# mzhaoshuai/CenterCLIP

Hardware: AMD Instinct MI355X
Metric: clips/sec (ViT-B/32, 12f) (higher is better)
Workload: dtype fp16 (MFMA operands; fp32 accumulate, residual stream, LN, softmax; cluster + similarity fp32); 1 GPU; cfg2 MSR-VTT-shaped: ViT-B/32 224^2, 12 frames -> 3 segments @block 7, K=49, batch 16, 32 words; global_batch=16, parallelism=single GPU

## Files before the change

### centerclip_amd/_lib_clip.py

```python
import ctypes as c

CC_MAX_LAYERS = 32
EPI = {"f16": 0, "f16_gelu": 1, "f32_resid": 2, "f32": 4}


class BlockWeights(c.Structure):
    _fields_ = [(n, c.c_void_p) for n in (
        "ln_1_weight", "ln_1_bias", "in_proj_weight_f16", "in_proj_bias", "out_proj_weight_f16", "out_proj_bias",
        "ln_2_weight", "ln_2_bias", "c_fc_weight_f16", "c_fc_bias", "c_proj_weight_f16", "c_proj_bias",
        "in_proj_ln_weight_f16", "in_proj_ln_c1", "in_proj_ln_c2", "c_fc_ln_weight_f16", "c_fc_ln_c1", "c_fc_ln_c2")]


class VitModel(c.Structure):
    _fields_ = [("layers", c.c_int32), ("width", c.c_int32), ("heads", c.c_int32), ("patch", c.c_int32),
                ("resolution", c.c_int32), ("embed_dim", c.c_int32),
                ("conv1_weight_f16", c.c_void_p), ("class_embedding", c.c_void_p),
                ("positional_embedding", c.c_void_p), ("ln_pre_weight", c.c_void_p), ("ln_pre_bias", c.c_void_p),
                ("ln_post_weight", c.c_void_p), ("ln_post_bias", c.c_void_p), ("proj", c.c_void_p),
                ("blocks", c.POINTER(BlockWeights)),
                ("cluster_frames", c.c_int32 * CC_MAX_LAYERS), ("cluster_tokens", c.c_int32 * CC_MAX_LAYERS),
                ("cluster_metric", c.c_int32), ("cluster_norm_p", c.c_float), ("cluster_threshold", c.c_float),
                ("cluster_iter_limit", c.c_int32), ("cluster_split_size", c.c_int32), ("cluster_pre_norm", c.c_int32),
                ("cluster_variants", c.c_void_p), ("row_policy", c.c_int32), ("conv2_weight_f16", c.c_void_p)]


class Frames(c.Structure):
    _fields_ = [("data", c.c_void_p), ("format", c.c_int32), ("mean", c.c_float * 3), ("std", c.c_float * 3)]


class TextModel(c.Structure):
    _fields_ = [("layers", c.c_int32), ("width", c.c_int32), ("heads", c.c_int32), ("context_length", c.c_int32),
                ("vocab_size", c.c_int32), ("embed_dim", c.c_int32),
                ("token_embedding", c.c_void_p), ("positional_embedding", c.c_void_p),
                ("ln_final_weight", c.c_void_p), ("ln_final_bias", c.c_void_p), ("text_projection", c.c_void_p),
                ("blocks", c.POINTER(BlockWeights)), ("row_policy", c.c_int32)]


ROWS_ALL_TEXT, ROWS_ALL_LAST_BLOCK = 1, 2


def declare(lib):
    vp, i32, i64, f32, sz = c.c_void_p, c.c_int32, c.c_int64, c.c_float, c.c_size_t
    lib.cc_linear_f16.argtypes = [vp, vp, vp, vp, i32, i32, i32, i32, i32, i32, vp]
    lib.cc_layernorm_f32.argtypes = [vp, i64, vp, vp, vp, i64, i32, i32, f32, i32, vp]
    lib.cc_attention_f16.argtypes = [vp, vp, i32, i32, i32, i32, i32, vp]
    lib.cc_fold_layernorm_linear_f32.argtypes = [vp, vp, vp, vp, i32, i32, vp, vp, vp, vp]
    lib.cc_fold_layernorm_linear_f32.restype = c.c_int
    lib.cc_row_stats_f16.argtypes = [vp, vp, vp, vp, i32, i32, vp]
    lib.cc_linear_ln_f16.argtypes = [vp, vp, vp, vp, vp, i32, f32, vp, i32, i32, i32, i32, i32, vp]
    lib.cc_linear_resid_stats_f16.argtypes = [vp, vp, vp, vp, vp, vp, c.POINTER(i32), vp, vp, i32, vp, i32, i32, i32, i32, vp]
    lib.cc_inproj_attention_f16.argtypes = [vp, vp, vp, vp, vp, i32, f32, vp, i32, i32, i32, i32, vp, vp, vp, vp]
    lib.cc_inproj_attention_f16.restype = c.c_int
    lib.cc_linear_tile_for.argtypes = [i32, i32, i32, i32]
    lib.cc_linear_tile_for.restype = c.c_int
    lib.cc_linear_resid_stats_slots.argtypes = [i32, i32, i32, i32]
    lib.cc_linear_resid_stats_slots.restype = c.c_int
    lib.cc_attention_strided_f16.argtypes = [vp, vp, i32, i32, i32, i32, i32, i64, i64, vp]
    lib.cc_attention_strided_f16.restype = c.c_int
    lib.cc_text_encode_hidden.argtypes = [c.POINTER(TextModel), vp, i32, i32, vp, vp, vp, sz, vp]
    lib.cc_text_encode_hidden.restype = c.c_int
    lib.cc_head_project_f32.argtypes = [vp, i32, vp, vp, vp, vp, vp, i32, i32, i32, vp]
    lib.cc_head_project_f32.restype = c.c_int
    lib.cc_contrastive_loss_f32.argtypes = [vp, i32, i64, i64, vp, vp, sz, vp]
    lib.cc_contrastive_loss_f32.restype = c.c_int
    lib.cc_contrastive_grad_workspace_bytes.argtypes = [i32, i32, i32]
    lib.cc_contrastive_grad_workspace_bytes.restype = sz
    lib.cc_contrastive_loss_grad_f32.argtypes = [vp, vp, vp, i64, i64, i32, i32, i32, f32, f32, vp, vp, vp, vp, vp, sz, vp]
    lib.cc_contrastive_loss_grad_f32.restype = c.c_int
    lib.cc_contrastive_loss_grad_dev_f32.argtypes = [vp, vp, vp, i64, i64, i32, i32, i32, f32, vp, f32, vp, vp, vp, vp, vp, sz, vp]
    lib.cc_contrastive_loss_grad_dev_f32.restype = c.c_int
    lib.cc_normalize_rows_f32.argtypes = [vp, vp, i32, i32, vp]
    lib.cc_normalize_rows_f32.restype = c.c_int
    lib.cc_loose_similarity_grouped_f32.argtypes = [vp, vp, vp, i32, i64, i64, i64, i64, i32, i32, i32, i32, f32, vp, i32,
                                                    vp, vp, sz, vp]
    lib.cc_loose_similarity_grouped_f32.restype = c.c_int
    for name in ("cc_row_stats_f16", "cc_linear_ln_f16", "cc_linear_resid_stats_f16"):
        getattr(lib, name).restype = c.c_int
    lib.cc_rank_counts_f32.argtypes = [vp, i32, i32, i64, i64, i32, vp, vp]
    lib.cc_rank_counts_f32.restype = c.c_int
    lib.cc_rank_counts_cols_f32.argtypes = [vp, i32, i32, i64, i64, vp, vp, vp]
    lib.cc_rank_counts_cols_f32.restype = c.c_int
# ... 118 lines not shown
```

### centerclip_amd/clip.py

```python
import contextlib
import ctypes
import torch
from torch import nn

import os

from . import _lib as L
from . import ops
from . import torch_ops as T
from ._lib_clip import BlockWeights, TextModel, VitModel, CC_MAX_LAYERS, ROWS_ALL_TEXT, ROWS_ALL_LAST_BLOCK
from .cluster import get_cluster_inter


PIXEL_MEAN = (0.48145466, 0.4578275, 0.40821073)
PIXEL_STD = (0.26862954, 0.26130258, 0.27577711)


def frames_descriptor(x, mean=PIXEL_MEAN, std=PIXEL_STD):
    from ._lib_clip import Frames
    fr = Frames()
    if x.dtype == torch.uint8:
        if x.ndim != 4 or (x.shape[1] != 3 and x.shape[-1] != 3):
            raise ValueError("uint8 frames must be [N,3,H,W] or [N,H,W,3], got %s" % (tuple(x.shape),))
        x = x.contiguous()
# ... 104 lines not shown
        out = self.resblocks((x, video_frame, cluster_loss))
        return out if visual else out[0]


class _Pack:

    def __init__(self):
        self.key = None
        self.keep = []
        self.struct = None
        self.handle = None

    @staticmethod
    def signature(module):
        return tuple((p.data_ptr(), p._version, str(p.device), p.dtype) for p in module.parameters())

    def f32(self, t):
        t = t.detach().float().contiguous()
        self.keep.append(t)
        return t.data_ptr()

    def f16(self, t):
        t = t.detach().to(torch.float16).contiguous()
        self.keep.append(t)
        return t.data_ptr()

    def fold(self, linear_w, linear_b, ln):
        w = linear_w.detach().float().contiguous()
        b = linear_b.detach().float().contiguous()
        gamma, beta = ln.weight.detach().float().contiguous(), ln.bias.detach().float().contiguous()
        N, K = w.shape
        wf = torch.empty(N, K, device=w.device, dtype=torch.float16)
        c1 = torch.empty(N, device=w.device, dtype=torch.float32)
        c2 = torch.empty(N, device=w.device, dtype=torch.float32)
        L.check(L.lib().cc_fold_layernorm_linear_f32(L.ptr(w), L.ptr(b), L.ptr(gamma), L.ptr(beta), N, K, L.ptr(wf),
                                                     L.ptr(c1), L.ptr(c2), L.stream_ptr(w.device)),
                "cc_fold_layernorm_linear_f32")
        self.keep += [wf, c1, c2]
        return wf.data_ptr(), c1.data_ptr(), c2.data_ptr()

    def blocks(self, transformer, count=None):
        arr = (BlockWeights * len(transformer.resblocks))()
        for i, blk in enumerate(transformer.resblocks):
            if count is not None and i >= count:
                break
            b = arr[i]
# ... 53 lines not shown
            (("prefix", int(n_blocks)),)
        if getattr(self, "_prefix_pack", None) is None:
            self._prefix_pack = _Pack()
        return self._build(self._prefix_pack, sig, int(n_blocks))

    def _build(self, pk, sig, n_blocks):
        if pk.key == sig:
            return pk.handle
        if pk.handle is not None:
            T.release_model(pk.handle)
        pk.keep, pk.key = [], sig
        m = VitModel()
        m.row_policy = ROWS_ALL_LAST_BLOCK if self.all_last_block_rows else 0
        m.layers, m.width, m.heads = self.transformer.layers, self.width, self.heads
        m.patch, m.resolution, m.embed_dim = self.patch_size, self.input_resolution, self.output_dim
        m.conv1_weight_f16 = pk.f16(self.conv1.weight.reshape(self.width, -1))
        if self.linear_patch == '3d':
            m.conv2_weight_f16 = pk.f16(self.conv2.weight.reshape(self.width, -1))
        m.class_embedding, m.positional_embedding = pk.f32(self.class_embedding), pk.f32(self.positional_embedding)
        m.ln_pre_weight, m.ln_pre_bias = pk.f32(self.ln_pre.weight), pk.f32(self.ln_pre.bias)
        if n_blocks is None:
            m.ln_post_weight, m.ln_post_bias = pk.f32(self.ln_post.weight), pk.f32(self.ln_post.bias)
            m.proj = pk.f32(self.proj)
        m.blocks = ctypes.cast(pk.blocks(self.transformer, n_blocks), ctypes.POINTER(BlockWeights))
        first = None
        tokens = (self.input_resolution // self.patch_size) ** 2
        variants = (L.ClusterVariant * CC_MAX_LAYERS)()
        any_variant = False
        dev = self.proj.device
        for i, blk in enumerate(self.transformer.resblocks):
            tc = blk.tokencluster_inter
            if tc is not None and tc.is_shift:
                m.cluster_frames[i], m.cluster_tokens[i] = tc.original_frame, tokens
                variants[i], keep = tc.variant(tokens, dev)
                pk.keep.extend(keep)
                any_variant = True
            elif tc is not None:
                m.cluster_frames[i], m.cluster_tokens[i] = tc.after_block_frames, tc.cluster_num
                if tc.algorithm == 'pooling' and tc.cluster_num != tokens:
                    raise ValueError("'pooling' keeps the token count: cluster_num_blocks[%d] must be %d" % (i, tokens))
                if getattr(tc, "mean_residual", False) and tc.cluster_num != tokens:
                    raise ValueError("mean_residual keeps the token count (cluster.py:229): cluster_num_blocks[%d] must be %d"
                                     % (i, tokens))
                variants[i], keep = tc.variant(tc.frame_duration * tokens, dev)
                pk.keep.extend(keep)
                any_variant = any_variant or not tc.is_default_variant
# ... 178 lines not shown
            hidden = hidden.view(h.shape[0], h.shape[1], -1)
            return hidden[:, 0, :], hidden
        feats, _ = self.visual.encode(image, video_frame)
        return feats, zero_scalar(image.device)

    def _text_model(self):
        tower = nn.ModuleList([self.transformer, self.token_embedding, self.ln_final])
        sig = _Pack.signature(tower) + ((self.positional_embedding._version, self.text_projection._version,
                                         self.positional_embedding.data_ptr(), self.text_projection.data_ptr(),
                                         bool(self.all_text_rows), bool(self.all_last_block_rows)),)
        pk = self._text_pack
        if pk.key == sig:
            return pk.handle
        if pk.handle is not None:
            T.release_model(pk.handle)
        pk.keep, pk.key = [], sig
        m = TextModel()
        m.row_policy = (ROWS_ALL_TEXT if self.all_text_rows else 0) | (ROWS_ALL_LAST_BLOCK if self.all_last_block_rows else 0)
        m.layers, m.width, m.heads = self.transformer.layers, self.transformer.width, self.transformer.heads
        m.context_length, m.vocab_size, m.embed_dim = self.context_length, self.vocab_size, self.embed_dim
        m.token_embedding, m.positional_embedding = pk.f32(self.token_embedding.weight), pk.f32(self.positional_embedding)
        m.ln_final_weight, m.ln_final_bias = pk.f32(self.ln_final.weight), pk.f32(self.ln_final.bias)
        m.text_projection = pk.f32(self.text_projection)
        m.blocks = ctypes.cast(pk.blocks(self.transformer), ctypes.POINTER(BlockWeights))
        pk.struct = m
        pk.handle = T.register_model(m, dict(embed_dim=self.embed_dim, width=self.transformer.width), pk)
        return pk.handle

    def text_prefix_parameters(self, n_blocks):
        ps = [self.token_embedding.weight, self.positional_embedding]
        for blk in list(self.transformer.resblocks)[:n_blocks]:
            ps += list(blk.parameters())
        return ps

    def _text_prefix_model(self, n_blocks):
        sig = tuple((p.data_ptr(), p._version, str(p.device), p.dtype) for p in self.text_prefix_parameters(n_blocks)) + \
            (("prefix", int(n_blocks)),)
        if getattr(self, "_text_prefix_pack", None) is None:
            self._text_prefix_pack = _Pack()
        pk = self._text_prefix_pack
        if pk.key == sig:
            return pk.handle
        if pk.handle is not None:
            T.release_model(pk.handle)
        pk.keep, pk.key = [], sig
        m = TextModel()
# ... 99 lines not shown
```

### centerclip_amd/csrc/cc_kernels.h

```cpp
#pragma once
#include "cc_common.h"

enum { EPI_F16 = 0, EPI_F16_GELU = 1, EPI_F32_RESID = 2, EPI_F32_PATCH = 3, EPI_F32 = 4,
       EPI_F16_LN = 5, EPI_F16_GELU_LN = 6, EPI_F32_RESID_STATS = 7,
       EPI_ATTN_LN = 8 };
#define CC_LN_MAX_SLOTS 32

struct GemmArgs {
    const _Float16* A;
    const _Float16* W;
    const float* bias;
    void* C;
    const float* R;
    const float* pos;
    int M, N, K, ldc;
    int lda, ldw;
    int patch_n;
    int tiles_m, tiles_n;
    const float* ln_stats;
    const float* ln_c1;
    int ln_slots;
    float ln_eps;
    float* stats_out;
    _Float16* c16;
    const float* shift_in;
    const float* shift_stats;
    int shift_slots;
    float* shift_out;
    const int* m_dev;
    int row_step;
    const int* row_map;
    float out_scale;
    int n_valid;
    const float* out_unscale_dev;
    int att_L, att_nseq, att_spt, att_causal;
    const int* att_seq_off;
    const int* att_seq_len;
};

struct GemmPair {
    GemmArgs p[2];
    int tiles0;
    int rider_prio;
};

int cc_gemm_dispatch(GemmArgs g, int epi, int tile, hipStream_t st);
int cc_gemm_dispatch2(GemmArgs g0, const GemmArgs* g1, int epi, int tile, hipStream_t st, int* slots_out = nullptr);
bool cc_gemm_timing_claim(const int rec12[12], hipEvent_t* start, hipEvent_t* stop);
bool cc_gemm_rows_ok(int N, int K, int epi);
int cc_gemm_rows_dispatch2(GemmArgs g0, const GemmArgs* g1, int epi, hipStream_t st, int* slots_out = nullptr);

struct LnArgs {
    const float* in; int64_t in_stride; const float* gamma; const float* beta; void* out; int64_t out_stride;
    int rows, W;
    _Float16* out16;
    float* stats;
    float* shift;
    const float* cls;
    const float* pos0;
    int cls_period;
};
struct TextEmbedArgs {
    const long long* ids; const float* tok_emb; const float* pos; float* h; int* eot; int Bt, Lt, W;
    _Float16* h16;
    float* stats;
    float* shift;
    int* seq_off;
    int* seq_len;
    int* m_total;
    int vocab;
};
int cc_launch_row_stats(const float* h, _Float16* h16, float* stats, float* shift, int rows, int W, hipStream_t st);
int cc_launch_layernorm2(const LnArgs& a0, const LnArgs* a1, float eps, int out_f16, hipStream_t st);
// ... 44 lines not shown
```

### centerclip_amd/csrc/clip_forward.hip

```cpp
#include "cc_kernels.h"
#include <cstdlib>
#include <cstdint>

namespace {

bool is_shift(const cc_cluster_variant* var) {
    return var && (var->algorithm == CC_CLUSTER_TEMPORAL_SHIFT || var->algorithm == CC_CLUSTER_TOKEN_SHIFT);
}

struct Carver {
    char* base;
    size_t off = 0;
    explicit Carver(void* b) : base(static_cast<char*>(b)) {}
    template <typename T>
    T* take(size_t count) {
        T* ptr = base ? reinterpret_cast<T*>(base + off) : nullptr;
        off += cc_align_up(count * sizeof(T), 256);
        return ptr;
    }
};

struct VitWs {
    _Float16* im2col;
    float* h;
// ... 46 lines not shown
    v.cluster = c.take<char>(cb);
    v.total = c.off;
    return v;
}

struct BlockCtx {
    float* h;
    _Float16* h16;
    float* st0;
    float* st1;
    float* sh0;
    float* sh1;
    _Float16* qkv;
    _Float16* att;
    _Float16* u;
    int nseq, L, W, heads, causal;
    int slots0, slots1;
    const int* m_dev;
    const int* seq_off;
    const int* seq_len;
    int sel_rows, sel_step;
    const int* sel_map;
    int mid_shift, mid_seg, mid_div;
};

int run_block_pair(const cc_block_weights* w0, BlockCtx* c0, const cc_block_weights* w1, BlockCtx* c1,
                   hipStream_t st) {
    if (!w0) { w0 = w1; c0 = c1; w1 = nullptr; c1 = nullptr; }
    const int M0 = c0->nseq * c0->L, M1 = c1 ? c1->nseq * c1->L : 0;
    const int Wa = c0->W, Wb = c1 ? c1->W : 0;
    int rc;
    int slots[2];
#ifdef CC_DEV_KNOBS
    static const int unpair_mask = [] { const char* e = getenv("CC_UNPAIR"); return e ? atoi(e) : 0; }();
#else
    constexpr int unpair_mask = 0;
#endif
    const int unpair = (c1 && M0 < 5000) ? unpair_mask : 0;
    auto dispatch = [&](GemmArgs& g0, GemmArgs& g1, int epi, int bit, int* sl) {
        if (!(unpair & bit)) return cc_gemm_dispatch2(g0, c1 ? &g1 : nullptr, epi, 0, st, sl);
        int s0[2] = {0, 0}, s1[2] = {0, 0};
        int r = cc_gemm_dispatch2(g0, nullptr, epi, 0, st, sl ? s0 : nullptr);
        if (r) return r;
        r = cc_gemm_dispatch2(g1, nullptr, epi, 0, st, sl ? s1 : nullptr);
        if (sl) { sl[0] = s0[0]; sl[1] = s1[0]; }
        return r;
    };
    auto base = [&](const BlockCtx* c, int M, const _Float16* A, const void* Wt, const float* bias, void* C, int N, int K) {
        GemmArgs g{};
        g.A = A; g.W = static_cast<const _Float16*>(Wt); g.bias = bias; g.C = C;
        g.M = M; g.N = N; g.K = K; g.ldc = N;
        g.ln_eps = 1e-5f;
        g.m_dev = c->m_dev;
        return g;
    };
    auto tail = [&](const BlockCtx* c, int M, const _Float16* A, const void* Wt, const float* bias, void* C, int N, int K) {
        GemmArgs g = base(c, M, A, Wt, bias, C, N, K);
        if (c->sel_rows > 0) { g.M = c->sel_rows; g.m_dev = nullptr; g.row_step = c->sel_step; g.row_map = c->sel_map; }
        return g;
    };
    auto tail_dispatch = [&](GemmArgs& g0, GemmArgs& g1, int epi, int bit, int* sl) {
        const bool s0 = c0->sel_rows > 0, s1 = c1 && c1->sel_rows > 0;
        if (!s0 && !s1) return dispatch(g0, g1, epi, bit, sl);
        if (s0 && (s1 || !c1)) return cc_gemm_rows_dispatch2(g0, c1 ? &g1 : nullptr, epi, st, sl);
        int a[2] = {0, 0}, b[2] = {0, 0};
        int* pa = sl ? a : nullptr;
        int* pb = sl ? b : nullptr;
        int r = s0 ? cc_gemm_rows_dispatch2(g0, nullptr, epi, st, pa) : cc_gemm_dispatch2(g0, nullptr, epi, 0, st, pa);
        if (r) return r;
        r = s1 ? cc_gemm_rows_dispatch2(g1, nullptr, epi, st, pb) : cc_gemm_dispatch2(g1, nullptr, epi, 0, st, pb);
        if (sl) { sl[0] = a[0]; sl[1] = b[0]; }
        return r;
    };
    {
        GemmArgs g0 = base(c0, M0, c0->h16, w0->in_proj_ln_weight_f16, w0->in_proj_ln_c2, c0->qkv, 3 * Wa, Wa);
        g0.ln_stats = c0->st0; g0.ln_slots = c0->slots0; g0.ln_c1 = w0->in_proj_ln_c1;
        GemmArgs g1{};
        if (c1) {
            g1 = base(c1, M1, c1->h16, w1->in_proj_ln_weight_f16, w1->in_proj_ln_c2, c1->qkv, 3 * Wb, Wb);
            g1.ln_stats = c1->st0; g1.ln_slots = c1->slots0; g1.ln_c1 = w1->in_proj_ln_c1;
        }
// ... 113 lines not shown
bool text_ok(const cc_text_model* m, int Lt) {
    return m->layers > 0 && m->layers <= CC_MAX_LAYERS && m->width == m->heads * 64 && Lt <= m->context_length;
}

int encode_towers(const cc_vit_model* vm, const cc_frames* video, int B, int T, float* vfeat, float* hidden_out,
                  int64_t* medoids_out, const int64_t* forced_medoids, const cc_text_model* tm, const int64_t* ids,
                  int Bt, int Lt, float* tfeat, float* text_hidden_out, void* ws, size_t ws_bytes, hipStream_t st,
                  int vstop = -1, int tstop = -1) {
    VitWs v{};
    TextWs t{};
    size_t off = 0;
    if (vm) { v = carve_vit(vm, B, T, ws); off = v.total; }
    if (tm) { t = carve_text(tm, Bt, Lt, static_cast<char*>(ws) + off); off += t.total; }
    if (!ws || ws_bytes < off) return CC_ERR_WORKSPACE;
    int rc = CC_OK;
    float* h = nullptr;
    float* hother = nullptr;
    int frames = T, tokens = 0, W = 0;
    const int vl = vm ? (vstop >= 0 ? vstop : vm->layers) : 0, tl = tm ? (tstop >= 0 ? tstop : tm->layers) : 0;
    const bool prefix = vstop >= 0 || tstop >= 0;
    const bool compact = tm && !text_hidden_out && Bt <= 256 && !(tm->row_policy & CC_ROWS_ALL_TEXT);
    BlockCtx cv{}, ct{};
    cv.slots0 = ct.slots0 = 1;
    if (tm) {
        ct.h = t.h; ct.h16 = t.h16; ct.st0 = t.st0; ct.st1 = t.st1; ct.sh0 = t.sh0; ct.sh1 = t.sh1;
        ct.qkv = t.qkv; ct.att = t.att; ct.u = t.u;
        ct.nseq = Bt; ct.L = Lt; ct.W = tm->width; ct.heads = tm->heads; ct.causal = 1;
        if (compact) { ct.m_dev = t.mcount; ct.seq_off = t.seq_off; ct.seq_len = t.seq_len; }
    }
    if (vm) {
        const int g = vm->resolution / vm->patch, n = g * g, F = B * T;
        W = vm->width;
        tokens = n;
        const bool patch3d = vm->conv2_weight_f16 != nullptr;
        rc = patch3d ? cc_launch_im2col3d(*video, v.im2col, F, T, vm->resolution, vm->patch, st)
                     : cc_launch_im2col(*video, v.im2col, F, vm->resolution, vm->patch, st);
        if (rc) return rc;
        GemmArgs ga{};
        ga.A = v.im2col;
        ga.W = static_cast<const _Float16*>(patch3d ? vm->conv2_weight_f16 : vm->conv1_weight_f16);
        ga.C = v.h;
        ga.pos = vm->positional_embedding;
        ga.M = F * n; ga.N = W; ga.K = (patch3d ? 9 : 3) * vm->patch * vm->patch; ga.ldc = W;
        ga.patch_n = n;
        rc = cc_gemm_dispatch(ga, EPI_F32_PATCH, 0, st);
        if (rc) return rc;
// ... 246 lines not shown
```

### centerclip_amd/csrc/gemm.hip

```cpp
#include "cc_kernels.h"
#include <hip/hip_ext.h>
#include <cstring>
#include <type_traits>
#include <unistd.h>
#include <cstdio>
#include <cstdlib>

typedef _Float16 h8 __attribute__((ext_vector_type(8)));
typedef _Float16 h4 __attribute__((ext_vector_type(4)));
typedef float f32x4 __attribute__((ext_vector_type(4)));

#define GEMM_BK 64
#ifdef CC_TWO_STAGES
#define GEMM_NST(BM, BN, WAVES, BK) 2
#else
#define GEMM_NST(BM, BN, WAVES, BK) (((WAVES) == 8 && (BK) == 64 && 3 * ((BM) + (BN)) * (BK) * 2 <= 160 * 1024) ? 3 : 2)
#endif

#define ATTN_QS 72
#define ATTN_VS 328
#define ATTN_Q_OFF 2048
#define ATTN_TAB_OFF (ATTN_Q_OFF + 2 * 256 * ATTN_QS * 2 + 64 * ATTN_VS * 2 + 8 * 16 * ATTN_QS * 2)
#define ATTN_SMEM (ATTN_TAB_OFF + 64 + 1024)

// ... 1302 lines not shown
        g.tiles_n = g.K / 64;
    };
    GemmPair pr{};
    shape(g0);
    pr.p[0] = g0;
    pr.tiles0 = g0.tiles_m * g0.tiles_n;
    int total = pr.tiles0;
    if (g1) {
        pr.p[1] = *g1;
        shape(pr.p[1]);
        total += pr.p[1].tiles_m * pr.p[1].tiles_n;
        pr.rider_prio = g0.M < 5000;
    } else {
        pr.p[1] = g0;
    }
    if (bm == 192) return launch_one<192, 192, 2, 4, EPI_ATTN_LN>(pr, total, st);
    if (bm == 224) return launch_one<224, 192, 2, 4, EPI_ATTN_LN>(pr, total, st);
    return launch_one<256, 192, 2, 4, EPI_ATTN_LN>(pr, total, st);
}

struct RowsPair {
    GemmArgs p[2];
    int blocks0;
};

constexpr int ROWS_BM = 64, ROWS_BN = 32, ROWS_WAVES = 8, ROWS_LDR = ROWS_BN + 4;

template <int EPI>
__global__ __launch_bounds__(64 * ROWS_WAVES) void gemm_rows_kernel(RowsPair pr) {
    const bool second = (int)blockIdx.x >= pr.blocks0;
    const GemmArgs g = second ? pr.p[1] : pr.p[0];
    const int bid = second ? blockIdx.x - pr.blocks0 : blockIdx.x;
    const int ncb = g.N / ROWS_BN;
    const int cb = bid % ncb, row0 = (bid / ncb) * ROWS_BM, col0 = cb * ROWS_BN;
    const int tid = threadIdx.x, wave = tid >> 6, lane = tid & 63, l15 = lane & 15, lg = lane >> 4;
    __shared__ float red[ROWS_WAVES / 2][ROWS_BM][ROWS_LDR];
    __shared__ float2 rowst[ROWS_BM];
    constexpr bool LNFOLD = (EPI == EPI_F16_GELU_LN);
    constexpr bool STATS = (EPI == EPI_F32_RESID_STATS);
    const int r = tid >> 3, sub = tid & 7, c = sub * 4;
    const int n = col0 + c;
    int mrow[5];
#pragma unroll
    for (int i = 0; i < 4; ++i) mrow[i] = min(row0 + i * 16 + l15, g.M - 1);
    mrow[4] = min(row0 + r, g.M - 1);
    int64_t prw[5];
    if (g.row_map) {
        int t[5];
#pragma unroll
        for (int i = 0; i < 5; ++i) t[i] = g.row_map[mrow[i]];
#pragma unroll
        for (int i = 0; i < 5; ++i) prw[i] = t[i];
    } else {
        const int step = g.row_step ? g.row_step : 1;
#pragma unroll
        for (int i = 0; i < 5; ++i) prw[i] = (int64_t)mrow[i] * step;
    }
    const int64_t pm = prw[4];
    const bool on = row0 + r < g.M;
    const int tsteps = g.K / 32, spw = (tsteps + ROWS_WAVES - 1) / ROWS_WAVES;
    const int kbeg = min(wave * spw, tsteps), ksteps = min(spw, tsteps - kbeg);
    const int klast = max(ksteps - 1, 0) * 32 + min(kbeg, tsteps - 1) * 32;
    const _Float16* wp[2];
    const _Float16* ap[4];
#pragma unroll
    for (int j = 0; j < 2; ++j) wp[j] = g.W + (int64_t)(col0 + j * 16 + l15) * g.K + lg * 8;
#pragma unroll
    for (int i = 0; i < 4; ++i) ap[i] = g.A + prw[i] * g.K + lg * 8;
    constexpr int U = 3;
    h8 bf[U][2], af[U][4];
    auto load_batch = [&](int s0) {
#pragma unroll
        for (int u = 0; u < U; ++u) {
            const int k = (s0 + u < ksteps) ? (kbeg + s0 + u) * 32 : klast;
#pragma unroll
            for (int j = 0; j < 2; ++j) bf[u][j] = *reinterpret_cast<const h8*>(wp[j] + k);
#pragma unroll
            for (int i = 0; i < 4; ++i) af[u][i] = *reinterpret_cast<const h8*>(ap[i] + k);
        }
    };
    load_batch(0);
    float2 t2[CC_LN_MAX_SLOTS / 8];
    float shin = 0.f;
    const bool rowscal = LNFOLD || (STATS && g.shift_stats);
    if (rowscal) {
        const int nslots = LNFOLD ? g.ln_slots : g.shift_slots;
        const float2* ps = reinterpret_cast<const float2*>(LNFOLD ? g.ln_stats : g.shift_stats) + pm * nslots;
#pragma unroll
        for (int u = 0; u < CC_LN_MAX_SLOTS / 8; ++u) t2[u] = ps[min(sub + u * 8, nslots - 1)];
        if (!LNFOLD && g.shift_in) shin = g.shift_in[pm];
    }
    const float4 bb = g.bias ? *reinterpret_cast<const float4*>(g.bias + n) : make_float4(0.f, 0.f, 0.f, 0.f);
// ... 52 lines not shown
    auto slot = [&](int i, int j) { return reinterpret_cast<float4*>(&red[wave & 3][i * 16 + l15][j * 16 + lg * 4]); };
    if (wave >= 4) {
#pragma unroll
        for (int i = 0; i < 4; ++i)
#pragma unroll
            for (int j = 0; j < 2; ++j) *slot(i, j) = make_float4(acc[i][j][0], acc[i][j][1], acc[i][j][2], acc[i][j][3]);
    }
    __syncthreads();
    if (wave < 4) {
#pragma unroll
        for (int i = 0; i < 4; ++i)
#pragma unroll
            for (int j = 0; j < 2; ++j) {
                const float4 t4 = *slot(i, j);
                *slot(i, j) = make_float4(acc[i][j][0] + t4.x, acc[i][j][1] + t4.y, acc[i][j][2] + t4.z, acc[i][j][3] + t4.w);
            }
    }
    __syncthreads();
    float4 v = make_float4(0.f, 0.f, 0.f, 0.f);
#pragma unroll
    for (int w = 0; w < ROWS_WAVES / 2; ++w) {
        const float4 t4 = *reinterpret_cast<const float4*>(&red[w][r][c]);
        v.x += t4.x; v.y += t4.y; v.z += t4.z; v.w += t4.w;
    }
    if (LNFOLD) {
        const float2 st = rowst[r];
        v.x = quick_gelu(st.y * (v.x - st.x * c1.x) + bb.x);
        v.y = quick_gelu(st.y * (v.y - st.x * c1.y) + bb.y);
        v.z = quick_gelu(st.y * (v.z - st.x * c1.z) + bb.z);
        v.w = quick_gelu(st.y * (v.w - st.x * c1.w) + bb.w);
        const h4 o = {(_Float16)v.x, (_Float16)v.y, (_Float16)v.z, (_Float16)v.w};
        if (on) *reinterpret_cast<h4*>(reinterpret_cast<_Float16*>(g.C) + pm * g.ldc + n) = o;
        return;
    }
    v.x += bb.x + res.x; v.y += bb.y + res.y; v.z += bb.z + res.z; v.w += bb.w + res.w;
    if (on) *reinterpret_cast<float4*>(reinterpret_cast<float*>(g.C) + pm * g.ldc + n) = v;
    if (STATS && g.c16) {
        const float cr = g.shift_stats ? rowst[r].x : 0.f;
        const h4 o = {(_Float16)(v.x - cr), (_Float16)(v.y - cr), (_Float16)(v.z - cr), (_Float16)(v.w - cr)};
        if (on) *reinterpret_cast<h4*>(g.c16 + pm * g.ldc + n) = o;
        if (on && g.shift_out && cb == 0 && c == 0) g.shift_out[pm] = cr;
        const float q0 = (float)o[0], q1 = (float)o[1], q2 = (float)o[2], q3 = (float)o[3];
        float psum = (q0 + q1) + (q2 + q3);
        float psq = (q0 * q0 + q1 * q1) + (q2 * q2 + q3 * q3);
        psum += dpp_f32<0xB1>(psum);
        psq += dpp_f32<0xB1>(psq);
        psum += dpp_f32<0x4E>(psum);
        psq += dpp_f32<0x4E>(psq);
        psum += dpp_f32<0x141>(psum);
        psq += dpp_f32<0x141>(psq);
        if (on && c == 0 && g.stats_out) reinterpret_cast<float2*>(g.stats_out)[pm * ncb + cb] = make_float2(psum, psq);
    }
}

bool cc_gemm_rows_ok(int N, int K, int epi) {
    if (N <= 0 || K <= 0 || (N % ROWS_BN) || (K % 32)) return false;
    if (epi == EPI_F32_RESID_STATS) return N / ROWS_BN <= CC_LN_MAX_SLOTS;
    return epi == EPI_F16_GELU_LN || epi == EPI_F32_RESID;
}

int cc_gemm_rows_dispatch2(GemmArgs g0, const GemmArgs* g1, int epi, hipStream_t st, int* slots_out) {
    if (!cc_gemm_rows_ok(g0.N, g0.K, epi) || (g1 && !cc_gemm_rows_ok(g1->N, g1->K, epi))) return CC_ERR_UNSUPPORTED;
    if (g0.M <= 0 || (g1 && g1->M <= 0)) return CC_ERR_INVALID;
    RowsPair pr{};
    pr.p[0] = g0;
    auto blocks = [](const GemmArgs& g) { return (g.N / ROWS_BN) * ((g.M + ROWS_BM - 1) / ROWS_BM); };
    pr.blocks0 = blocks(g0);
    int total = pr.blocks0;
    if (g1) { pr.p[1] = *g1; total += blocks(*g1); }
    if (slots_out) { slots_out[0] = g0.N / ROWS_BN; slots_out[1] = g1 ? g1->N / ROWS_BN : 0; }
    const dim3 grid(total), block(64 * ROWS_WAVES);
    switch (epi) {
        case EPI_F16_GELU_LN: hipLaunchKernelGGL(gemm_rows_kernel<EPI_F16_GELU_LN>, grid, block, 0, st, pr); break;
        case EPI_F32_RESID: hipLaunchKernelGGL(gemm_rows_kernel<EPI_F32_RESID>, grid, block, 0, st, pr); break;
        case EPI_F32_RESID_STATS: hipLaunchKernelGGL(gemm_rows_kernel<EPI_F32_RESID_STATS>, grid, block, 0, st, pr); break;
        default: return CC_ERR_UNSUPPORTED;
    }
    return hipGetLastError() == hipSuccess ? CC_OK : CC_ERR_HIP;
}

int cc_gemm_dispatch(GemmArgs g, int epi, int tile, hipStream_t st) { return cc_gemm_dispatch2(g, nullptr, epi, tile, st, nullptr); }

extern "C" {

int cc_linear_unscaled_f16(const void* a_f16, const void* w_f16, float* c, int32_t M, int32_t N, int32_t K,
                           const float* scale_dev, void* stream) {
    if (!a_f16 || !w_f16 || !c || !scale_dev) return CC_ERR_INVALID;
    GemmArgs g{};
    g.A = static_cast<const _Float16*>(a_f16);
    g.W = static_cast<const _Float16*>(w_f16);
    g.C = c;
    g.M = M; g.N = N; g.K = K; g.ldc = N;
    g.out_unscale_dev = scale_dev;
    return cc_gemm_dispatch(g, EPI_F32, 0, static_cast<hipStream_t>(stream));
}
int cc_linear_f16(const void* a_f16, const void* w_f16, const float* bias, void* c, int32_t M, int32_t N, int32_t K,
                  int32_t ldc, int32_t epilogue, int32_t tile, void* stream) {
    if (!a_f16 || !w_f16 || !c) return CC_ERR_INVALID;
// ... 71 lines not shown
}

int cc_linear_resid_stats_f16(const void* a_f16, const void* w_f16, const float* bias, float* h, void* h16_out,
                              float* stats_out, int32_t* slots_out, const float* shift_in, const float* stats_in,
                              int32_t slots_in, float* shift_out, int32_t M, int32_t N, int32_t K, int32_t tile,
                              void* stream) {
    if (!a_f16 || !w_f16 || !h || !h16_out || !stats_out || !slots_out) return CC_ERR_INVALID;
    if (stats_in && (slots_in <= 0 || slots_in > CC_LN_MAX_SLOTS || !shift_out)) return CC_ERR_INVALID;
    GemmArgs g{};
    g.A = static_cast<const _Float16*>(a_f16);
    g.W = static_cast<const _Float16*>(w_f16);
    g.bias = bias;
    g.C = h;
    g.M = M; g.N = N; g.K = K; g.ldc = N;
    g.c16 = static_cast<_Float16*>(h16_out);
    g.stats_out = stats_out;
    g.shift_in = shift_in; g.shift_stats = stats_in; g.shift_slots = slots_in; g.shift_out = shift_out;
    int slots[2] = {0, 0};
    const int rc = cc_gemm_dispatch2(g, nullptr, EPI_F32_RESID_STATS, tile, static_cast<hipStream_t>(stream), slots);
    *slots_out = slots[0];
    return rc;
}

int cc_debug_gemm_timing_begin(int cap) {
    if (g_timing.ev) {
        for (int i = 0; i < 2 * g_timing.cap; ++i) (void)hipEventDestroy(g_timing.ev[i]);
        delete[] g_timing.ev;
        delete[] g_timing.info;
        g_timing = GemmTiming{};
    }
    if (cap <= 0) return CC_OK;
    g_timing.ev = new hipEvent_t[2 * cap];
    g_timing.info = new int[cap][12];
    for (int i = 0; i < 2 * cap; ++i)
        if (hipEventCreate(&g_timing.ev[i]) != hipSuccess) return CC_ERR_HIP;
    g_timing.cap = cap;
    g_timing.armed = true;
    return CC_OK;
}

int cc_debug_gemm_timing_end(void) {
    g_timing.armed = false;
    return g_timing.count;
}

int cc_debug_gemm_timing_read(int i, float* us_out, int* info12_out) {
// ... 10 lines not shown
```

### include/centerclip_hip.h

```cpp
#ifndef CENTERCLIP_HIP_H
#define CENTERCLIP_HIP_H

#include <stddef.h>
#include <stdint.h>

#ifdef __cplusplus
extern "C" {
#endif

typedef enum cc_status {
    CC_OK = 0,
    CC_ERR_INVALID = -1,
    CC_ERR_UNSUPPORTED = -2,
    CC_ERR_WORKSPACE = -3,
    CC_ERR_HIP = -4
} cc_status;

#define CC_KMEDOIDS_MAX_THRESHOLD 1e-5f

#define CC_METRIC_EUCLIDEAN 0
#define CC_METRIC_COSINE 1

const char* cc_version(void);
const char* cc_status_string(int status);
// ... 175 lines not shown
                                 int32_t N, int32_t K, void* w_f16_out, float* c1_out, float* c2_out, void* stream);

#define CC_MAX_LAYERS 32

#define CC_ROWS_ALL_TEXT        1
#define CC_ROWS_ALL_LAST_BLOCK  2

typedef struct cc_vit_model {
    int32_t layers, width, heads, patch, resolution, embed_dim;
    const void* conv1_weight_f16;
    const float* class_embedding;
    const float* positional_embedding;
    const float* ln_pre_weight;  const float* ln_pre_bias;
    const float* ln_post_weight; const float* ln_post_bias;
    const float* proj;
    const cc_block_weights* blocks;
    int32_t cluster_frames[CC_MAX_LAYERS];
    int32_t cluster_tokens[CC_MAX_LAYERS];
    int32_t cluster_metric;   float cluster_norm_p;   float cluster_threshold;
    int32_t cluster_iter_limit, cluster_split_size, cluster_pre_norm;
    const struct cc_cluster_variant* cluster_variants;
    int32_t row_policy;
    const void* conv2_weight_f16;
} cc_vit_model;

#define CC_FRAMES_F32_CHW 0
#define CC_FRAMES_U8_CHW  1
#define CC_FRAMES_U8_HWC  2
typedef struct cc_frames {
    const void* data;
    int32_t format;
    float mean[3], std[3];
} cc_frames;

size_t cc_vit_workspace_bytes(const cc_vit_model* m, int32_t B, int32_t T);

int64_t cc_vit_forced_medoids_count(const cc_vit_model* m, int32_t B);

int cc_vit_encode(const cc_vit_model* m, const float* video, int32_t B, int32_t T,
                  float* features, float* hidden_out, int64_t* medoids_out,
                  const int64_t* forced_medoids, void* ws, size_t ws_bytes, void* stream);

typedef struct cc_text_model {
    int32_t layers, width, heads, context_length, vocab_size, embed_dim;
    const float* token_embedding;
    const float* positional_embedding;
    const float* ln_final_weight; const float* ln_final_bias;
    const float* text_projection;
    const cc_block_weights* blocks;
    int32_t row_policy;
} cc_text_model;

size_t cc_text_workspace_bytes(const cc_text_model* m, int32_t Bt, int32_t Lt);

int cc_text_encode(const cc_text_model* m, const int64_t* ids, int32_t Bt, int32_t Lt,
                   float* features, void* ws, size_t ws_bytes, void* stream);
int cc_text_encode_hidden(const cc_text_model* m, const int64_t* ids, int32_t Bt, int32_t Lt,
                          float* features, float* hidden_out, void* ws, size_t ws_bytes, void* stream);

int cc_head_project_f32(const float* h, int32_t row_mul, const int32_t* row_idx, const float* gamma,
                        const float* beta, const float* proj, float* out, int32_t R, int32_t W, int32_t E,
                        void* stream);

size_t cc_clip_workspace_bytes(const cc_vit_model* vm, int32_t B, int32_t T,
                               const cc_text_model* tm, int32_t Bt, int32_t Lt);
int cc_clip_encode(const cc_vit_model* vm, const float* video, int32_t B, int32_t T,
                   float* visual_features, int64_t* medoids_out,
                   const cc_text_model* tm, const int64_t* ids, int32_t Bt, int32_t Lt,
                   float* text_features, void* ws, size_t ws_bytes, void* stream);

int cc_vit_encode_frames(const cc_vit_model* m, const cc_frames* frames, int32_t B, int32_t T,
                         float* features, float* hidden_out, int64_t* medoids_out,
                         const int64_t* forced_medoids, void* ws, size_t ws_bytes, void* stream);
int cc_clip_encode_frames(const cc_vit_model* vm, const cc_frames* frames, int32_t B, int32_t T,
                          float* visual_features, int64_t* medoids_out, const int64_t* forced_medoids,
                          const cc_text_model* tm, const int64_t* ids, int32_t Bt, int32_t Lt,
                          float* text_features, void* ws, size_t ws_bytes, void* stream);

int cc_vit_encode_prefix_frames(const cc_vit_model* m, const cc_frames* frames, int32_t B, int32_t T, int32_t n_blocks,
                                float* hidden_out, const int64_t* forced_medoids, void* ws, size_t ws_bytes,
                                void* stream);
// ... 151 lines not shown
```

Baseline: 8795 clips/s.

## Add split-K with ticketed slab reduction to the selected-rows GEMM kernel

The row-selected tail GEMM (last-block selected rows, compact text rows) now splits the K dimension across several workgroups per output tile when the tile count is small. Partial sums go to a global scratch slab, and the last-arriving workgroup, chosen by an atomic ticket counter, reduces them and runs the epilogue. This targets low occupancy on the few-tile tail GEMMs. In exchange it adds global scratch traffic, fences and atomics, plus a persistent scratch buffer per model.

```diff
diff --git a/centerclip_amd/_lib_clip.py b/centerclip_amd/_lib_clip.py
--- a/centerclip_amd/_lib_clip.py
+++ b/centerclip_amd/_lib_clip.py
@@ -21,7 +21,8 @@
                 ("cluster_frames", c.c_int32 * CC_MAX_LAYERS), ("cluster_tokens", c.c_int32 * CC_MAX_LAYERS),
                 ("cluster_metric", c.c_int32), ("cluster_norm_p", c.c_float), ("cluster_threshold", c.c_float),
                 ("cluster_iter_limit", c.c_int32), ("cluster_split_size", c.c_int32), ("cluster_pre_norm", c.c_int32),
-                ("cluster_variants", c.c_void_p), ("row_policy", c.c_int32), ("conv2_weight_f16", c.c_void_p)]
+                ("cluster_variants", c.c_void_p), ("row_policy", c.c_int32), ("conv2_weight_f16", c.c_void_p),
+                ("rows_scratch", c.c_void_p)]
 
 
 class Frames(c.Structure):
@@ -33,7 +34,15 @@
                 ("vocab_size", c.c_int32), ("embed_dim", c.c_int32),
                 ("token_embedding", c.c_void_p), ("positional_embedding", c.c_void_p),
                 ("ln_final_weight", c.c_void_p), ("ln_final_bias", c.c_void_p), ("text_projection", c.c_void_p),
-                ("blocks", c.POINTER(BlockWeights)), ("row_policy", c.c_int32)]
+                ("blocks", c.POINTER(BlockWeights)), ("row_policy", c.c_int32), ("rows_scratch", c.c_void_p)]
+
+
+class RowsProblem(c.Structure):
+    _fields_ = [("a_f16", c.c_void_p), ("w_f16", c.c_void_p), ("bias", c.c_void_p), ("c", c.c_void_p),
+                ("M", c.c_int32), ("N", c.c_int32), ("K", c.c_int32), ("row_step", c.c_int32), ("row_map", c.c_void_p),
+                ("ln_stats", c.c_void_p), ("ln_slots", c.c_int32), ("ln_c1", c.c_void_p), ("ln_eps", c.c_float),
+                ("c16", c.c_void_p), ("stats_out", c.c_void_p), ("shift_in", c.c_void_p), ("shift_stats", c.c_void_p),
+                ("shift_slots", c.c_int32), ("shift_out", c.c_void_p), ("scratch", c.c_void_p)]
 
 
 ROWS_ALL_TEXT, ROWS_ALL_LAST_BLOCK = 1, 2
@@ -57,6 +66,11 @@
     lib.cc_linear_resid_stats_slots.restype = c.c_int
     lib.cc_attention_strided_f16.argtypes = [vp, vp, i32, i32, i32, i32, i32, i64, i64, vp]
     lib.cc_attention_strided_f16.restype = c.c_int
+    for name, args, res in (("cc_rows_scratch_bytes", [], sz),
+                            ("cc_linear_rows_f16", [c.POINTER(RowsProblem), c.POINTER(RowsProblem), i32, i32, vp], c.c_int),
+                            ("cc_linear_rows_plan", [i32, i32, i32, i32, i32, i32, i32, c.POINTER(i32)], c.c_int)):
+        if hasattr(lib, name):
+            getattr(lib, name).argtypes, getattr(lib, name).restype = args, res
     lib.cc_text_encode_hidden.argtypes = [c.POINTER(TextModel), vp, i32, i32, vp, vp, vp, sz, vp]
     lib.cc_text_encode_hidden.restype = c.c_int
     lib.cc_head_project_f32.argtypes = [vp, i32, vp, vp, vp, vp, vp, i32, i32, i32, vp]
diff --git a/centerclip_amd/clip.py b/centerclip_amd/clip.py
--- a/centerclip_amd/clip.py
+++ b/centerclip_amd/clip.py
@@ -150,6 +150,14 @@
 
     def f16(self, t):
         t = t.detach().to(torch.float16).contiguous()
+        self.keep.append(t)
+        return t.data_ptr()
+
+    def rows_scratch(self, device):
+        lib = L.lib()
+        if not hasattr(lib, "cc_rows_scratch_bytes"):
+            return None
+        t = torch.zeros(lib.cc_rows_scratch_bytes(), device=device, dtype=torch.uint8)
         self.keep.append(t)
         return t.data_ptr()
 
@@ -249,6 +257,7 @@
         if n_blocks is None:
             m.ln_post_weight, m.ln_post_bias = pk.f32(self.ln_post.weight), pk.f32(self.ln_post.bias)
             m.proj = pk.f32(self.proj)
+            m.rows_scratch = pk.rows_scratch(self.proj.device)
         m.blocks = ctypes.cast(pk.blocks(self.transformer, n_blocks), ctypes.POINTER(BlockWeights))
         first = None
         tokens = (self.input_resolution // self.patch_size) ** 2
@@ -473,6 +482,7 @@
         m.token_embedding, m.positional_embedding = pk.f32(self.token_embedding.weight), pk.f32(self.positional_embedding)
         m.ln_final_weight, m.ln_final_bias = pk.f32(self.ln_final.weight), pk.f32(self.ln_final.bias)
         m.text_projection = pk.f32(self.text_projection)
+        m.rows_scratch = pk.rows_scratch(self.text_projection.device)
         m.blocks = ctypes.cast(pk.blocks(self.transformer), ctypes.POINTER(BlockWeights))
         pk.struct = m
         pk.handle = T.register_model(m, dict(embed_dim=self.embed_dim, width=self.transformer.width), pk)
diff --git a/centerclip_amd/csrc/cc_kernels.h b/centerclip_amd/csrc/cc_kernels.h
--- a/centerclip_amd/csrc/cc_kernels.h
+++ b/centerclip_amd/csrc/cc_kernels.h
@@ -30,6 +30,7 @@
     const int* m_dev;
     int row_step;
     const int* row_map;
+    void* rows_scratch;
     float out_scale;
     int n_valid;
     const float* out_unscale_dev;
@@ -48,7 +49,9 @@
 int cc_gemm_dispatch2(GemmArgs g0, const GemmArgs* g1, int epi, int tile, hipStream_t st, int* slots_out = nullptr);
 bool cc_gemm_timing_claim(const int rec12[12], hipEvent_t* start, hipEvent_t* stop);
 bool cc_gemm_rows_ok(int N, int K, int epi);
-int cc_gemm_rows_dispatch2(GemmArgs g0, const GemmArgs* g1, int epi, hipStream_t st, int* slots_out = nullptr);
+int cc_gemm_rows_dispatch2(GemmArgs g0, const GemmArgs* g1, int epi, hipStream_t st, int* slots_out = nullptr,
+                           int force_slices = 0);
+int cc_gemm_rows_plan(const int M[2], const int N[2], const int K[2], const bool scratch[2], int force, int S[2]);
 
 struct LnArgs {
     const float* in; int64_t in_stride; const float* gamma; const float* beta; void* out; int64_t out_stride;
diff --git a/centerclip_amd/csrc/clip_forward.hip b/centerclip_amd/csrc/clip_forward.hip
--- a/centerclip_amd/csrc/clip_forward.hip
+++ b/centerclip_amd/csrc/clip_forward.hip
@@ -92,6 +92,7 @@
     int sel_rows, sel_step;
     const int* sel_map;
     int mid_shift, mid_seg, mid_div;
+    void* rows_scratch;
 };
 
 int run_block_pair(const cc_block_weights* w0, BlockCtx* c0, const cc_block_weights* w1, BlockCtx* c1,
@@ -126,7 +127,10 @@
     };
     auto tail = [&](const BlockCtx* c, int M, const _Float16* A, const void* Wt, const float* bias, void* C, int N, int K) {
         GemmArgs g = base(c, M, A, Wt, bias, C, N, K);
-        if (c->sel_rows > 0) { g.M = c->sel_rows; g.m_dev = nullptr; g.row_step = c->sel_step; g.row_map = c->sel_map; }
+        if (c->sel_rows > 0) {
+            g.M = c->sel_rows; g.m_dev = nullptr; g.row_step = c->sel_step; g.row_map = c->sel_map;
+            g.rows_scratch = c->rows_scratch;
+        }
         return g;
     };
     auto tail_dispatch = [&](GemmArgs& g0, GemmArgs& g1, int epi, int bit, int* sl) {
@@ -286,6 +290,8 @@
     const bool compact = tm && !text_hidden_out && Bt <= 256 && !(tm->row_policy & CC_ROWS_ALL_TEXT);
     BlockCtx cv{}, ct{};
     cv.slots0 = ct.slots0 = 1;
+    cv.rows_scratch = vm ? vm->rows_scratch : nullptr;
+    ct.rows_scratch = tm ? tm->rows_scratch : nullptr;
     if (tm) {
         ct.h = t.h; ct.h16 = t.h16; ct.st0 = t.st0; ct.st1 = t.st1; ct.sh0 = t.sh0; ct.sh1 = t.sh1;
         ct.qkv = t.qkv; ct.att = t.att; ct.u = t.u;
diff --git a/centerclip_amd/csrc/gemm.hip b/centerclip_amd/csrc/gemm.hip
--- a/centerclip_amd/csrc/gemm.hip
+++ b/centerclip_amd/csrc/gemm.hip
@@ -1348,17 +1348,25 @@
 struct RowsPair {
     GemmArgs p[2];
     int blocks0;
+    int S[2];
 };
 
 constexpr int ROWS_BM = 64, ROWS_BN = 32, ROWS_WAVES = 8, ROWS_LDR = ROWS_BN + 4;
-
-template <int EPI>
+constexpr int ROWS_BATCH = 3;
+constexpr int ROWS_ROUND = 256;
+constexpr int ROWS_TICKETS = 256;
+constexpr size_t ROWS_SLAB = (size_t)ROWS_BM * ROWS_BN;
+
+template <int EPI, bool SPLIT>
 __global__ __launch_bounds__(64 * ROWS_WAVES) void gemm_rows_kernel(RowsPair pr) {
     const bool second = (int)blockIdx.x >= pr.blocks0;
     const GemmArgs g = second ? pr.p[1] : pr.p[0];
     const int bid = second ? blockIdx.x - pr.blocks0 : blockIdx.x;
     const int ncb = g.N / ROWS_BN;
-    const int cb = bid % ncb, row0 = (bid / ncb) * ROWS_BM, col0 = cb * ROWS_BN;
+    const int S = SPLIT ? (second ? pr.S[1] : pr.S[0]) : 1;
+    const int ntiles = ncb * ((g.M + ROWS_BM - 1) / ROWS_BM);
+    const int slice = SPLIT ? bid / ntiles : 0, tile = SPLIT ? bid % ntiles : bid;
+    const int cb = tile % ncb, row0 = (tile / ncb) * ROWS_BM, col0 = cb * ROWS_BN;
     const int tid = threadIdx.x, wave = tid >> 6, lane = tid & 63, l15 = lane & 15, lg = lane >> 4;
     __shared__ float red[ROWS_WAVES / 2][ROWS_BM][ROWS_LDR];
     __shared__ float2 rowst[ROWS_BM];
@@ -1385,7 +1393,13 @@
     const int64_t pm = prw[4];
     const bool on = row0 + r < g.M;
     const int tsteps = g.K / 32, spw = (tsteps + ROWS_WAVES - 1) / ROWS_WAVES;
-    const int kbeg = min(wave * spw, tsteps), ksteps = min(spw, tsteps - kbeg);
+    int kbeg = min(wave * spw, tsteps), ksteps = min(spw, tsteps - kbeg);
+    if (SPLIT && S > 1) {
+        const int sb = tsteps / S, sr = tsteps % S, ssteps = sb + (slice < sr);
+        const int wb = ssteps / ROWS_WAVES, wr = ssteps % ROWS_WAVES;
+        kbeg = slice * sb + min(slice, sr) + wave * wb + min(wave, wr);
+        ksteps = wb + (wave < wr);
+    }
     const int klast = max(ksteps - 1, 0) * 32 + min(kbeg, tsteps - 1) * 32;
     const _Float16* wp[2];
     const _Float16* ap[4];
@@ -1393,7 +1407,7 @@
     for (int j = 0; j < 2; ++j) wp[j] = g.W + (int64_t)(col0 + j * 16 + l15) * g.K + lg * 8;
 #pragma unroll
     for (int i = 0; i < 4; ++i) ap[i] = g.A + prw[i] * g.K + lg * 8;
-    constexpr int U = 3;
+    constexpr int U = ROWS_BATCH;
     h8 bf[U][2], af[U][4];
     auto load_batch = [&](int s0) {
 #pragma unroll
@@ -1492,6 +1506,34 @@
     for (int w = 0; w < ROWS_WAVES / 2; ++w) {
         const float4 t4 = *reinterpret_cast<const float4*>(&red[w][r][c]);
         v.x += t4.x; v.y += t4.y; v.z += t4.z; v.w += t4.w;
+    }
+    if (SPLIT && S > 1) {
+        unsigned* tickets = static_cast<unsigned*>(g.rows_scratch);
+        float* slabs = reinterpret_cast<float*>(tickets + ROWS_TICKETS) + (size_t)tile * S * ROWS_SLAB;
+        *reinterpret_cast<float4*>(slabs + slice * ROWS_SLAB + tid * 4) = v;
+        asm volatile("s_waitcnt vmcnt(0)" ::: "memory");
+        __syncthreads();
+        int* flag = reinterpret_cast<int*>(&red[0][0][0]);
+        if (tid == 0) {
+            __builtin_amdgcn_fence(__ATOMIC_RELEASE, "agent");
+            asm volatile("s_waitcnt vmcnt(0)" ::: "memory");
+            const unsigned t = __hip_atomic_fetch_add(tickets + tile, 1u, __ATOMIC_RELAXED, __HIP_MEMORY_SCOPE_AGENT);
+            const bool last = t == (unsigned)(S - 1);
+            if (last) {
+                __builtin_amdgcn_fence(__ATOMIC_ACQUIRE, "agent");
+                asm volatile("s_waitcnt vmcnt(0)" ::: "memory");
+                __hip_atomic_store(tickets + tile, 0u, __ATOMIC_RELAXED, __HIP_MEMORY_SCOPE_AGENT);
+            }
+            *flag = last;
+        }
+        __syncthreads();
+        if (!*flag) return;
+        v = make_float4(0.f, 0.f, 0.f, 0.f);
+#pragma unroll 4
+        for (int s = 0; s < S; ++s) {
+            const float4 t4 = *reinterpret_cast<const float4*>(slabs + s * ROWS_SLAB + tid * 4);
+            v.x += t4.x; v.y += t4.y; v.z += t4.z; v.w += t4.w;
+        }
     }
     if (LNFOLD) {
         const float2 st = rowst[r];
@@ -1529,21 +1571,46 @@
     return epi == EPI_F16_GELU_LN || epi == EPI_F32_RESID;
 }
 
-int cc_gemm_rows_dispatch2(GemmArgs g0, const GemmArgs* g1, int epi, hipStream_t st, int* slots_out) {
+int cc_gemm_rows_plan(const int M[2], const int N[2], const int K[2], const bool scratch[2], int force, int S[2]) {
+    int tiles[2] = {0, 0};
+    for (int i = 0; i < 2; ++i) tiles[i] = M[i] > 0 ? (N[i] / ROWS_BN) * ((M[i] + ROWS_BM - 1) / ROWS_BM) : 0;
+    const int round = max(1, ROWS_ROUND / (tiles[0] + tiles[1]));
+    int total = 0;
+    for (int i = 0; i < 2; ++i) {
+        S[i] = 1;
+        if (!tiles[i]) continue;
+        const int tsteps = K[i] / 32, batch = ROWS_WAVES * ROWS_BATCH;
+        const int want = force > 0 ? force : min((tsteps + batch - 1) / batch, round);
+        const int by_k = tsteps / ROWS_WAVES, by_scratch = scratch[i] ? min(ROWS_TICKETS, ROWS_ROUND) / tiles[i] : 1;
+        S[i] = max(1, min(want, min(by_k, by_scratch)));
+        total += S[i] * tiles[i];
+    }
+    return total;
+}
+
+template <int EPI>
+static void rows_launch(const RowsPair& pr, int total, bool split, hipStream_t st) {
+    const dim3 grid(total), block(64 * ROWS_WAVES);
+    if (split) hipLaunchKernelGGL((gemm_rows_kernel<EPI, true>), grid, block, 0, st, pr);
+    else hipLaunchKernelGGL((gemm_rows_kernel<EPI, false>), grid, block, 0, st, pr);
+}
+
+int cc_gemm_rows_dispatch2(GemmArgs g0, const GemmArgs* g1, int epi, hipStream_t st, int* slots_out, int force_slices) {
     if (!cc_gemm_rows_ok(g0.N, g0.K, epi) || (g1 && !cc_gemm_rows_ok(g1->N, g1->K, epi))) return CC_ERR_UNSUPPORTED;
     if (g0.M <= 0 || (g1 && g1->M <= 0)) return CC_ERR_INVALID;
     RowsPair pr{};
     pr.p[0] = g0;
-    auto blocks = [](const GemmArgs& g) { return (g.N / ROWS_BN) * ((g.M + ROWS_BM - 1) / ROWS_BM); };
-    pr.blocks0 = blocks(g0);
-    int total = pr.blocks0;
-    if (g1) { pr.p[1] = *g1; total += blocks(*g1); }
+    if (g1) pr.p[1] = *g1;
+    const int M[2] = {g0.M, g1 ? g1->M : 0}, N[2] = {g0.N, g1 ? g1->N : 0}, K[2] = {g0.K, g1 ? g1->K : 0};
+    const bool scratch[2] = {g0.rows_scratch != nullptr, g1 && g1->rows_scratch && g1->rows_scratch != g0.rows_scratch};
+    const int total = cc_gemm_rows_plan(M, N, K, scratch, force_slices, pr.S);
+    pr.blocks0 = pr.S[0] * (g0.N / ROWS_BN) * ((g0.M + ROWS_BM - 1) / ROWS_BM);
     if (slots_out) { slots_out[0] = g0.N / ROWS_BN; slots_out[1] = g1 ? g1->N / ROWS_BN : 0; }
-    const dim3 grid(total), block(64 * ROWS_WAVES);
+    const bool split = pr.S[0] > 1 || pr.S[1] > 1;
     switch (epi) {
-        case EPI_F16_GELU_LN: hipLaunchKernelGGL(gemm_rows_kernel<EPI_F16_GELU_LN>, grid, block, 0, st, pr); break;
-        case EPI_F32_RESID: hipLaunchKernelGGL(gemm_rows_kernel<EPI_F32_RESID>, grid, block, 0, st, pr); break;
-        case EPI_F32_RESID_STATS: hipLaunchKernelGGL(gemm_rows_kernel<EPI_F32_RESID_STATS>, grid, block, 0, st, pr); break;
+        case EPI_F16_GELU_LN: rows_launch<EPI_F16_GELU_LN>(pr, total, split, st); break;
+        case EPI_F32_RESID: rows_launch<EPI_F32_RESID>(pr, total, split, st); break;
+        case EPI_F32_RESID_STATS: rows_launch<EPI_F32_RESID_STATS>(pr, total, split, st); break;
         default: return CC_ERR_UNSUPPORTED;
     }
     return hipGetLastError() == hipSuccess ? CC_OK : CC_ERR_HIP;
@@ -1661,6 +1728,53 @@
     return rc;
 }
 
+size_t cc_rows_scratch_bytes(void) { return ROWS_TICKETS * sizeof(unsigned) + ROWS_ROUND * ROWS_SLAB * sizeof(float); }
+
+int cc_linear_rows_plan(int32_t M0, int32_t N0, int32_t K0, int32_t M1, int32_t N1, int32_t K1, int32_t epilogue,
+                        int32_t* slices_out) {
+    if (!slices_out || M0 <= 0 || M1 < 0 || !cc_gemm_rows_ok(N0, K0, epilogue) || (M1 > 0 && !cc_gemm_rows_ok(N1, K1, epilogue)))
+        return CC_ERR_INVALID;
+    const int M[2] = {M0, M1}, N[2] = {N0, M1 > 0 ? N1 : 0}, K[2] = {K0, M1 > 0 ? K1 : 0};
+    const bool scratch[2] = {true, true};
+    int S[2];
+    const int total = cc_gemm_rows_plan(M, N, K, scratch, 0, S);
+    slices_out[0] = S[0];
+    slices_out[1] = M1 > 0 ? S[1] : 0;
+    return total;
+}
+
+static bool rows_problem_args(const cc_rows_problem* p, int epi, GemmArgs* out) {
+    if (!p->a_f16 || !p->w_f16 || !p->c || p->M <= 0 || p->row_step < 0) return false;
+    GemmArgs g{};
+    g.A = static_cast<const _Float16*>(p->a_f16);
+    g.W = static_cast<const _Float16*>(p->w_f16);
+    g.bias = p->bias;
+    g.C = p->c;
+    g.M = p->M; g.N = p->N; g.K = p->K; g.ldc = p->N;
+    g.row_step = p->row_step; g.row_map = p->row_map;
+    g.rows_scratch = p->scratch;
+    if (epi == EPI_F16_GELU_LN) {
+        if (!p->ln_stats || !p->ln_c1 || p->ln_slots <= 0 || p->ln_slots > CC_LN_MAX_SLOTS) return false;
+        g.ln_stats = p->ln_stats; g.ln_slots = p->ln_slots; g.ln_c1 = p->ln_c1; g.ln_eps = p->ln_eps;
+    } else if (epi == EPI_F32_RESID_STATS) {
+        if (!p->c16 || !p->stats_out) return false;
+        if (p->shift_stats && (p->shift_slots <= 0 || p->shift_slots > CC_LN_MAX_SLOTS || !p->shift_out)) return false;
+        g.c16 = static_cast<_Float16*>(p->c16); g.stats_out = p->stats_out;
+        g.shift_in = p->shift_in; g.shift_stats = p->shift_stats; g.shift_slots = p->shift_slots; g.shift_out = p->shift_out;
+    }
+    *out = g;
+    return true;
+}
+
+int cc_linear_rows_f16(const cc_rows_problem* p0, const cc_rows_problem* p1, int32_t epilogue, int32_t force_slices,
+                       void* stream) {
+    if (!p0 || force_slices < 0) return CC_ERR_INVALID;
+    if (epilogue != EPI_F16_GELU_LN && epilogue != EPI_F32_RESID && epilogue != EPI_F32_RESID_STATS) return CC_ERR_UNSUPPORTED;
+    GemmArgs g0{}, g1{};
+    if (!rows_problem_args(p0, epilogue, &g0) || (p1 && !rows_problem_args(p1, epilogue, &g1))) return CC_ERR_INVALID;
+    return cc_gemm_rows_dispatch2(g0, p1 ? &g1 : nullptr, epilogue, static_cast<hipStream_t>(stream), nullptr, force_slices);
+}
+
 int cc_debug_gemm_timing_begin(int cap) {
     if (g_timing.ev) {
         for (int i = 0; i < 2 * g_timing.cap; ++i) (void)hipEventDestroy(g_timing.ev[i]);
diff --git a/include/centerclip_hip.h b/include/centerclip_hip.h
--- a/include/centerclip_hip.h
+++ b/include/centerclip_hip.h
@@ -221,6 +221,7 @@
     const struct cc_cluster_variant* cluster_variants;
     int32_t row_policy;
     const void* conv2_weight_f16;
+    void* rows_scratch;
 } cc_vit_model;
 
 #define CC_FRAMES_F32_CHW 0
@@ -248,6 +249,7 @@
     const float* text_projection;
     const cc_block_weights* blocks;
     int32_t row_policy;
+    void* rows_scratch;
 } cc_text_model;
 
 size_t cc_text_workspace_bytes(const cc_text_model* m, int32_t Bt, int32_t Lt);
@@ -256,6 +258,21 @@
                    float* features, void* ws, size_t ws_bytes, void* stream);
 int cc_text_encode_hidden(const cc_text_model* m, const int64_t* ids, int32_t Bt, int32_t Lt,
                           float* features, float* hidden_out, void* ws, size_t ws_bytes, void* stream);
+
+typedef struct cc_rows_problem {
+    const void* a_f16; const void* w_f16; const float* bias; void* c;
+    int32_t M, N, K;
+    int32_t row_step; const int32_t* row_map;
+    const float* ln_stats; int32_t ln_slots; const float* ln_c1; float ln_eps;
+    void* c16; float* stats_out;
+    const float* shift_in; const float* shift_stats; int32_t shift_slots; float* shift_out;
+    void* scratch;
+} cc_rows_problem;
+size_t cc_rows_scratch_bytes(void);
+int cc_linear_rows_f16(const cc_rows_problem* p0, const cc_rows_problem* p1, int32_t epilogue, int32_t force_slices,
+                       void* stream);
+int cc_linear_rows_plan(int32_t M0, int32_t N0, int32_t K0, int32_t M1, int32_t N1, int32_t K1, int32_t epilogue,
+                        int32_t* slices_out);
 
 int cc_head_project_f32(const float* h, int32_t row_mul, const int32_t* row_idx, const float* gamma,
                         const float* beta, const float* proj, float* out, int32_t R, int32_t W, int32_t E,
```

Measured after the change: 8769 clips/s. Within noise of the previous version (-0.3%).
